# 10XGenomics/vartrix

Hardware: NVIDIA B200
Metric: reads_sw_scored_per_sec (higher is better)
Workload: dtype int16x2

## Files before the change

vartrix_b200/csrc/vtx_api.cu:

```cuda
#include "../../include/vartrix_b200.h"
#include "vtx_pipeline.cuh"
#include "vtx_sw.cuh"
#include "vtx_sw_band.cuh"
#include "vtx_inflate.cuh"
#include "vtx_stage.cuh"

#include <nvtx3/nvToolsExt.h>

#include <algorithm>
#include <cstdarg>
#include <cstdio>
#include <cstring>
#include <string>
#include <thread>
#include <vector>

using namespace vtx;

namespace {

thread_local std::string g_create_error;

struct Nvtx {
    explicit Nvtx(const char* name) { nvtxRangePushA(name); }
// ... 71 lines not shown
    void* h_res[7] = { nullptr, nullptr, nullptr, nullptr, nullptr, nullptr, nullptr };
    size_t h_res_cap = 0;
    void* h_scalars = nullptr;
    uint64_t last_n = 0;
    vtx_metrics last_metrics{};

    cudaStream_t fetch_stream = nullptr;
    unsigned long long* h_cum = nullptr;
    unsigned long long* d_cum = nullptr;
    std::vector<TimeRec> trecs;
    size_t trec_used = 0;
    bool timing_valid = false;
    uint32_t last_tiles_nl = 0;
    bool last_tiles_valid = false;
    uint64_t t_pairs = 0;

    void* comm = nullptr;
    int rank = 0, n_ranks = 1;
    void* g_host[7] = { nullptr, nullptr, nullptr, nullptr, nullptr, nullptr, nullptr };
    size_t g_host_cap = 0;
    DBuf g_dev[7];
    DBuf g_counts;
    cudaStream_t comm_stream = nullptr;
    cudaEvent_t ev_counts = nullptr, ev_gather = nullptr, ev_results = nullptr;
    uint64_t* h_counts = nullptr;
    bool gather_pending = false;
    bool gather_guard = false;
    vtx_result g_out{};
};

namespace {

int set_err(vtx_ctx* c, int code, const char* fmt, ...)
{
    char buf[512];
    va_list ap; va_start(ap, fmt); vsnprintf(buf, sizeof(buf), fmt, ap); va_end(ap);
    if (c) c->err = buf; else g_create_error = buf;
    return code;
}

#define CK(call)                                                                                     \
    do {                                                                                             \
        cudaError_t e_ = (call);                                                                     \
        if (e_ != cudaSuccess)                                                                       \
            return set_err(ctx, VTX_E_CUDA, "%s failed: %s (%s:%d)", #call, cudaGetErrorString(e_), __FILE__, __LINE__); \
    } while (0)

int ensure(vtx_ctx* ctx, DBuf& b, size_t bytes)
{
    if (bytes <= b.cap) return VTX_OK;
    if (b.p) {
        CK(cudaStreamSynchronize(ctx->stream));
        if (ctx->copy_stream) CK(cudaStreamSynchronize(ctx->copy_stream));
        CK(cudaFree(b.p)); b.p = nullptr; b.cap = 0;
    }
    size_t want = bytes + bytes / 8 + 256;
    cudaError_t e = cudaMalloc(&b.p, want);
    if (e != cudaSuccess) { b.p = nullptr; return set_err(ctx, VTX_E_NOMEM, "cudaMalloc(%zu) failed: %s", want, cudaGetErrorString(e)); }
    b.cap = want;
    return VTX_OK;
}

#define ENS(buf, bytes) do { int rc_ = ensure(ctx, buf, (bytes)); if (rc_) return rc_; } while (0)

template <typename T> T* P(DBuf& b) { return static_cast<T*>(b.p); }

TimeRec* new_trec(vtx_ctx* ctx)
{
    if (ctx->finished) ctx->trec_used = 0;
    if (ctx->trec_used == ctx->trecs.size()) {
        TimeRec r;
        for (auto& e : r.ev) if (cudaEventCreate(&e) != cudaSuccess) return nullptr;
        ctx->trecs.push_back(r);
    }
    TimeRec* r = &ctx->trecs[ctx->trec_used++];
    r->had_h2d = false; r->sw_launches = 0; r->launches = 0;
    return r;
}

inline unsigned blocks_for(uint64_t n, unsigned threads) { return unsigned((n + threads - 1) / threads); }

int scan_u32(vtx_ctx* ctx, const uint32_t* in, uint64_t n, uint32_t* out, uint64_t* launches)
{
    const unsigned nb = std::max(1u, blocks_for(n, kScanTile));
    ENS(ctx->scan_sums, size_t(nb) * 4);
    vtx_k_scan_tiles<<<nb, kScanThreads, 0, ctx->stream>>>(in, n, out, P<uint32_t>(ctx->scan_sums));
    vtx_k_scan_sums<<<1, kScanThreads, 0, ctx->stream>>>(P<uint32_t>(ctx->scan_sums), nb, out + n);
    vtx_k_scan_add<<<nb, kScanThreads, 0, ctx->stream>>>(out, n, P<uint32_t>(ctx->scan_sums));
    if (launches) *launches += 3;
    CK(cudaGetLastError());
    return VTX_OK;
}

struct DevBatch {
    uint32_t n_loci = 0; uint32_t n_reads = 0; uint64_t n_cand = 0;
    const uint32_t* locus_row; const uint8_t* hap; const uint32_t *ref_off, *ref_len, *alt_off, *alt_len;
    const uint64_t* cand_start; const uint8_t* read_nib; const uint64_t* read_off; const uint32_t* read_len;
    const uint8_t* cb_bytes; const uint32_t* read_cb_off; const uint16_t* read_cb_len; const uint64_t* read_umi;
    const uint32_t* cand_read;
    const uint64_t* read_cb_key = nullptr; const uint32_t* cb_off_ex = nullptr;
    uint32_t class_mask = ~0u;
    uint32_t max_read_len = 0, max_hap_len = 0;
    uint64_t max_depth = ~0ull;
};

struct SwAllow { bool split, multi, fold; };
SwAllow sw_allow(const vtx_ctx* ctx, uint32_t max_read, uint32_t max_hap)
{
    SwAllow a;
    a.split = max_read <= uint32_t(kSplitMaxRead) && !(ctx->cfg.flags & VTX_F_NO_SPLIT);
    a.multi = max_read <= uint32_t(kMultiMaxRead) && max_hap > uint32_t(class_max_n(kNumFastClasses - 1));
    a.fold = !(ctx->cfg.flags & (VTX_F_NO_SPLIT | VTX_F_NO_FOLD));
    return a;
}
template <int CLS>
int launch_sw_class(vtx_ctx* ctx, SwArgs a, uint64_t* launches)
{
    using TC = TileClass<CLS>;
    constexpr int PPW = 32 / TC::LPP, RS = TC::LPP * TC::CS;
    const size_t codes_bytes = (size_t(PPW) * (a.mcap + 2 * TC::LPP) * 2 + 7) & ~size_t(7);
    const size_t bnd_bytes = (CLS == kMultiClass && a.multi) ? size_t(PPW) * (a.mcap + 8) * 8 : 0;
    const size_t warp_bytes = (size_t(5 * RS) * 4 + codes_bytes + bnd_bytes + 15) & ~size_t(15);
    constexpr int kSwThreads = TC::THREADS;
    const size_t smem = warp_bytes * (kSwThreads / 32);
    auto kern = vtx_k_sw_pairs<CLS>;
    CK(cudaFuncSetAttribute(kern, cudaFuncAttributeMaxDynamicSharedMemorySize, int(smem)));
    int per_sm = 0;
    CK(cudaOccupancyMaxActiveBlocksPerMultiprocessor(&per_sm, kern, kSwThreads, smem));
    if (per_sm < 1) return set_err(ctx, VTX_E_CUDA, "SW kernel class %d does not fit on an SM (smem %zu)", CLS, smem);
    kern<<<ctx->n_sm * per_sm, kSwThreads, smem, ctx->stream>>>(a);
    CK(cudaGetLastError());
    ++*launches;
    return VTX_OK;
}

template <int SCLS>
int launch_sw_split(vtx_ctx* ctx, SwArgs a, uint64_t* launches)
{
    using SC = SplitClass<SCLS>;
    const size_t smem = split_warp_bytes<SCLS>(a.mcap) * (SC::THREADS / 32);
    auto kern = vtx_k_sw_split<SCLS>;
    CK(cudaFuncSetAttribute(kern, cudaFuncAttributeMaxDynamicSharedMemorySize, int(smem)));
    int per_sm = 0;
    CK(cudaOccupancyMaxActiveBlocksPerMultiprocessor(&per_sm, kern, SC::THREADS, smem));
    if (per_sm < 1) return set_err(ctx, VTX_E_CUDA, "split SW kernel %d does not fit on an SM (smem %zu)", SCLS, smem);
    kern<<<ctx->n_sm * per_sm, SC::THREADS, smem, ctx->stream>>>(a);
    CK(cudaGetLastError());
    ++*launches;
    return VTX_OK;
}

int launch_sw_fold(vtx_ctx* ctx, SwArgs a, uint64_t* launches)
{
    const size_t smem = fold_warp_bytes() * (kFoldThreads / 32);
    auto kern = vtx_k_sw_fold;
    CK(cudaFuncSetAttribute(kern, cudaFuncAttributeMaxDynamicSharedMemorySize, int(smem)));
    int per_sm = 0;
    CK(cudaOccupancyMaxActiveBlocksPerMultiprocessor(&per_sm, kern, kFoldThreads, smem));
    if (per_sm < 1) return set_err(ctx, VTX_E_CUDA, "folded SW kernel does not fit on an SM (smem %zu)", smem);
    kern<<<ctx->n_sm * per_sm, kFoldThreads, smem, ctx->stream>>>(a);
    CK(cudaGetLastError());
    ++*launches;
    return VTX_OK;
}

int run_sw(vtx_ctx* ctx, const DevBatch& b, uint32_t n_pairs_ub, const uint32_t* pair_slot, uint32_t* counters,
           uint32_t* pair_scores, uint64_t* launches, uint64_t* sw_launches, TimeRec* tr)
{
    const uint32_t nl = b.n_loci;
    ENS(ctx->tcount, size_t(kNumClasses) * (nl + 1) * 4);
    ENS(ctx->tstart, size_t(kNumClasses) * (nl + 1) * 4);
    ENS(ctx->tile_counters, 64);
    const int force_slow = 0;
    const SwAllow allow = sw_allow(ctx, b.max_read_len, b.max_hap_len);
    const int allow_split = allow.split, allow_multi = allow.multi, allow_fold = allow.fold;
    vtx_k_locus_prep<<<blocks_for(uint64_t(nl) * 32, 256), 256, 0, ctx->stream>>>(
        nl, b.hap, b.ref_off, b.ref_len, b.alt_off, b.alt_len, P<uint32_t>(ctx->pair_start), P<uint32_t>(ctx->pair_read), b.read_len,
        force_slow, allow_split, allow_multi, allow_fold, b.max_read_len, b.max_hap_len, P<unsigned long long>(ctx->d_metrics) + 4,
        P<uint32_t>(ctx->tcount));
    ++*launches;
    vtx_k_scan_rows<<<kNumClasses, kScanThreads, 0, ctx->stream>>>(P<uint32_t>(ctx->tcount), P<uint32_t>(ctx->tstart), nl, nl + 1);
    ++*launches;
    CK(cudaGetLastError());
    CK(cudaMemsetAsync(ctx->tile_counters.p, 0, 64, ctx->stream));
    ctx->last_tiles_nl = nl;
    ctx->last_tiles_valid = true;
    if (tr) CK(cudaEventRecord(tr->ev[EV_PREP], ctx->stream));

    SwArgs a{};
    a.hap_bytes = b.hap; a.ref_off = b.ref_off; a.ref_len = b.ref_len; a.alt_off = b.alt_off; a.alt_len = b.alt_len;
    a.read_nib = b.read_nib; a.read_off = b.read_off; a.read_len = b.read_len;
    a.pair_read = P<uint32_t>(ctx->pair_read); a.pair_start = P<uint32_t>(ctx->pair_start);
    a.n_loci = nl; a.pair_slot = pair_slot; a.counters = counters; a.pair_scores = pair_scores;
    a.min_score = ctx->cfg.min_score;
    int mcap = int(std::min<uint32_t>(b.max_read_len, kFastMaxRead));
    mcap = std::max(2, (mcap + 1) & ~1);
    a.mcap = mcap;
    a.k64k = 65536u;
    a.one = 1u;
    a.multi = allow_multi;
    a.max_hap = b.max_hap_len;

    uint64_t before = *launches;
    if (ctx->cfg.band_mode == VTX_BAND_MODEL) {
        BandArgs ba{};
        ba.sw = a; ba.n_pairs_ub = n_pairs_ub; ba.k = ctx->cfg.band_k; ba.w = ctx->cfg.band_w;
        ba.max_read = std::max<uint32_t>(b.max_read_len, 8); ba.max_hap = std::max<uint32_t>(b.max_hap_len, 8);
        const uint64_t all_hits = uint64_t(ba.max_read) * ba.max_hap;
        ba.hit_cap = uint32_t(std::min<uint64_t>(all_hits, uint64_t(1) << 20));
        ba.hit_cap = std::min<uint32_t>(ba.hit_cap, 65535u * 16u);
        const size_t wb = band_warp_bytes(ba.max_read, ba.max_hap, ba.hit_cap);
        size_t warps = size_t(ctx->n_sm) * 16;
        const size_t budget = size_t(4) << 30;
        if (warps * wb > budget) warps = std::max<size_t>(size_t(ctx->n_sm), budget / wb);
        warps = std::max<size_t>(warps & ~size_t(3), 4);
        ENS(ctx->band_scratch, warps * wb);
        ba.scratch = P<uint8_t>(ctx->band_scratch);
        if (ba.max_hap >= 65536u || ba.max_read >= 65536u) return set_err(ctx, VTX_E_UNSUPPORTED, "band model: reads and windows must be shorter than 65536");
        ba.overflow = P<unsigned long long>(ctx->d_metrics) + 5;
        ba.bounds_violated = P<unsigned long long>(ctx->d_metrics) + 4;
        ba.cursor = P<uint32_t>(ctx->tile_counters);
        vtx_k_sw_band<<<unsigned(warps / (kBandThreads / 32)), kBandThreads, 0, ctx->stream>>>(ba);
        CK(cudaGetLastError());
        ++*launches;
        *sw_launches += *launches - before;
        return VTX_OK;
    }
    for (int c = 0; c < kNumFastClasses; ++c) {
        if (c > 0 && b.max_hap_len <= uint32_t(class_max_n(c - 1))) continue;
        if (!(b.class_mask >> c & 1u)) continue;
        a.tile_start = P<uint32_t>(ctx->tstart) + size_t(c) * (nl + 1);
        a.tile_counter = P<uint32_t>(ctx->tile_counters) + c;
        int rc = VTX_OK;
        switch (c) {
        case 0: rc = launch_sw_class<0>(ctx, a, launches); break;
        case 1: rc = launch_sw_class<1>(ctx, a, launches); break;
        case 2: rc = launch_sw_class<2>(ctx, a, launches); break;
        case 3: rc = launch_sw_class<3>(ctx, a, launches); break;
        }
        if (rc) return rc;
    }
    if (allow_split) {
        for (int c = 0; c < kNumSplitClasses; ++c) {
            if (c > 0 && b.max_hap_len <= uint32_t(split_max_n(c - 1))) continue;
            if (!(b.class_mask >> (kSplitClass0 + c) & 1u)) continue;
            a.tile_start = P<uint32_t>(ctx->tstart) + size_t(kSplitClass0 + c) * (nl + 1);
            a.tile_counter = P<uint32_t>(ctx->tile_counters) + kSplitClass0 + c;
            int rc = c == 0 ? launch_sw_split<0>(ctx, a, launches) : launch_sw_split<1>(ctx, a, launches);
            if (rc) return rc;
        }
    }
    if (allow_fold && (b.class_mask >> kFoldClass & 1u)) {
        a.tile_start = P<uint32_t>(ctx->tstart) + size_t(kFoldClass) * (nl + 1);
        a.tile_counter = P<uint32_t>(ctx->tile_counters) + kFoldClass;
        int rc = launch_sw_fold(ctx, a, launches);
        if (rc) return rc;
    }
    if (b.class_mask >> kSlowClass & 1u) {
        const unsigned blocks = unsigned(ctx->n_sm) * 4, threads = 128;
        const size_t warps = size_t(blocks) * threads / 32;
        ENS(ctx->scratch, warps * (size_t(b.max_hap_len) + 1) * 32 * 4);
        a.scratch = P<uint32_t>(ctx->scratch);
        a.tile_start = P<uint32_t>(ctx->tstart) + size_t(kSlowClass) * (nl + 1);
        a.tile_counter = P<uint32_t>(ctx->tile_counters) + kSlowClass;
        vtx_k_sw_generic<<<blocks, threads, 0, ctx->stream>>>(a);
        CK(cudaGetLastError());
        ++*launches;
    }
    *sw_launches += *launches - before;
    (void)n_pairs_ub;
    return VTX_OK;
}

int grow_results(vtx_ctx* ctx, size_t need)
{
    if (need <= ctx->res_cap) return VTX_OK;
    const size_t ncap = need + need / 4 + 1024;
    DBuf* bufs[7] = { &ctx->r_row, &ctx->r_col, &ctx->r_ref, &ctx->r_alt, &ctx->r_unk, &ctx->r_val, &ctx->r_val2 };
    const size_t esz[7] = { 4, 4, 4, 4, 4, 8, 8 };
    for (int i = 0; i < 7; ++i) {
        void* np = nullptr;
        cudaError_t e = cudaMalloc(&np, ncap * esz[i]);
        if (e != cudaSuccess) return set_err(ctx, VTX_E_NOMEM, "result cudaMalloc(%zu) failed: %s", ncap * esz[i], cudaGetErrorString(e));
        if (bufs[i]->p && ctx->res_ub && !ctx->finished)
            CK(cudaMemcpyAsync(np, bufs[i]->p, ctx->res_ub * esz[i], cudaMemcpyDeviceToDevice, ctx->stream));
        if (bufs[i]->p) {
            CK(cudaStreamSynchronize(ctx->stream));
            if (ctx->fetch_stream) CK(cudaStreamSynchronize(ctx->fetch_stream));
            if (ctx->comm_stream) CK(cudaStreamSynchronize(ctx->comm_stream));
            CK(cudaFree(bufs[i]->p));
        }
        bufs[i]->p = np; bufs[i]->cap = ncap * esz[i];
    }
    ctx->res_cap = ncap;
    return VTX_OK;
}

int process_batch(vtx_ctx* ctx, const DevBatch& b, TimeRec* tr)
{
    const uint64_t nc = b.n_cand;
    const uint32_t nl = b.n_loci, nr = b.n_reads;
    const int use_umi = ctx->cfg.use_umi ? 1 : 0;
    uint64_t launches = 0, sw_launches = 0;
    cudaStream_t st = ctx->stream;

    if (ctx->finished) {
        CK(cudaMemsetAsync(ctx->d_res_n.p, 0, 8, st));
        CK(cudaMemsetAsync(ctx->d_metrics.p, 0, 48, st));
        ctx->res_ub = 0;
        ctx->finished = false;
    }
    int rc = grow_results(ctx, ctx->res_ub + nc);
    if (rc) return rc;
// ... 1345 lines not shown
```

vartrix_b200/csrc/vtx_sw.cuh:

```cuda
#pragma once
#include <cstdint>
#include <cuda_runtime.h>

namespace vtx {

constexpr int kMatch = 1, kMismatch = -5, kGapOpen = -5, kGapExtend = -1;
constexpr int kGoe = kGapOpen + kGapExtend;

__host__ __device__ constexpr uint32_t pack2(int lo, int hi)
{
    return (uint32_t(uint16_t(int16_t(hi))) << 16) | uint32_t(uint16_t(int16_t(lo)));
}
constexpr int kBias = 16384;
constexpr uint32_t kGE2 = pack2(kGapExtend, kGapExtend);
constexpr uint32_t kBIAS2 = pack2(kBias, kBias);
constexpr uint32_t kGOE2 = pack2(kBias + kGoe, kBias + kGoe);
constexpr uint32_t kNEG2 = pack2(0, 0);
constexpr uint32_t kGoeAdd = (uint32_t(uint16_t(int16_t(kGoe - 1))) << 16) | uint32_t(uint16_t(int16_t(kGoe)));
#ifndef VTX_SW_FUSE
#define VTX_SW_FUSE 1
#endif
#ifndef VTX_SW_HADD
#define VTX_SW_HADD 0
#endif
__device__ __forceinline__ uint32_t padd(uint32_t x, uint32_t one, uint32_t c)
{
    (void)one;
    return x + c;
}
__device__ __forceinline__ uint32_t hadd(uint32_t h, uint32_t one, int col)
{
#if VTX_SW_HADD == 1
    (void)col;
    return h * one + kGoeAdd;
#elif VTX_SW_HADD == 2
    return (col & 1) ? h + kGoeAdd : h * one + kGoeAdd;
#else
    (void)one; (void)col;
    return h + kGoeAdd;
#endif
}
__device__ __forceinline__ uint32_t sw_h(uint32_t diag, uint32_t one, uint32_t s, uint32_t f, uint32_t e)
{
#if VTX_SW_FUSE
    (void)one;
    return __vimax3_s16x2(__viaddmax_s16x2(diag, s, f), e, kBIAS2);
#else
    return __vmaxs2(__vimax3_s16x2(padd(diag, one, s), f, kBIAS2), e);
#endif
}
constexpr int kProfMatch = kMatch - kGoe, kProfMis = kMismatch - kGoe;

constexpr int kFastMaxRead = 1024;
constexpr int kMaxRead = 16000;
constexpr int kNumFastClasses = 4;
constexpr int kSlowClass = kNumFastClasses;
constexpr int kNumSplitClasses = 2;
constexpr int kSplitClass0 = kSlowClass + 1;
constexpr int kFoldClass = kSplitClass0 + kNumSplitClasses;
constexpr int kNumClasses = kFoldClass + 1;
constexpr int kTileChunk = 8;

template <int CLS> struct TileClass;
template <> struct TileClass<0> { static constexpr int LPP = 8, C = 26, CS = 28, THREADS = 320, MINB = 2; };
template <> struct TileClass<1> { static constexpr int LPP = 8, C = 29, CS = 36, THREADS = 320, MINB = 2; };
template <> struct TileClass<2> { static constexpr int LPP = 8, C = 32, CS = 36, THREADS = 256, MINB = 2; };
template <> struct TileClass<3> { static constexpr int LPP = 8, C = 40, CS = 44, THREADS = 384, MINB = 1; };
constexpr int kMultiClass = 3;
constexpr int kMultiMaxRead = 256;
__host__ __device__ constexpr int class_max_n(int cls)
{
    return cls == 0 ? 208 : cls == 1 ? 232 : cls == 2 ? 256 : cls == 3 ? 320 : 0x7fffffff;
}
constexpr int kSlowPairsPerWarp = 16;

struct SwArgs {
    const uint8_t* hap_bytes;
    const uint32_t* ref_off; const uint32_t* ref_len; const uint32_t* alt_off; const uint32_t* alt_len;
    const uint8_t* read_nib; const uint64_t* read_off; const uint32_t* read_len;
    const uint32_t* pair_read;
    const uint32_t* pair_start;
    const uint32_t* tile_start;
    uint32_t n_loci;
    uint32_t* tile_counter;
    const uint32_t* pair_slot;
    uint32_t* counters;
    uint32_t* pair_scores;
    int32_t min_score;
    int32_t mcap;
    uint32_t k64k;
    uint32_t one;
    int32_t multi;
    uint32_t* scratch;
    uint32_t max_hap;
};

__device__ __forceinline__ uint32_t hap_code(uint8_t b)
{
    return b == 'A' ? 0u : b == 'C' ? 1u : b == 'G' ? 2u : b == 'T' ? 3u : 5u;
}
__device__ __forceinline__ uint32_t nib_code(uint32_t nib)
{
    return (0x4444444344424104ull >> (nib * 4)) & 0xF;
}

__device__ __forceinline__ uint32_t upper_locus(const uint32_t* __restrict__ a, uint32_t n, uint32_t v)
{
    uint32_t lo = 0, hi = n;
    while (hi - lo > 1) {
        uint32_t mid = (lo + hi) >> 1;
        if (__ldg(a + mid) <= v) lo = mid; else hi = mid;
    }
    return lo;
}

__device__ __forceinline__ void call_and_scatter(const SwArgs& a, uint32_t pair, uint32_t packed)
{
    const int ref_score = int(int16_t(packed & 0xFFFF)), alt_score = int(int16_t(packed >> 16));
    if (a.pair_scores) a.pair_scores[pair] = pack2(ref_score, alt_score);
    if (!a.pair_slot) return;
    if (ref_score < a.min_score && alt_score < a.min_score) return;
    const uint32_t k = ref_score > alt_score ? 0u : (alt_score > ref_score ? 1u : 2u);
    atomicAdd(a.counters + size_t(a.pair_slot[pair]) * 4 + k, 1u);
}

template <int CLS>
__global__ void __launch_bounds__(TileClass<CLS>::THREADS, TileClass<CLS>::MINB) vtx_k_sw_pairs(const SwArgs a)
{
    using TC = TileClass<CLS>;
    constexpr int LPP = TC::LPP, C = TC::C, CS = TC::CS;
    constexpr int PPW = 32 / LPP;
    constexpr int RS = LPP * CS;
    constexpr int M = LPP;
    static_assert(CS % 4 == 0 && ((CS / 4) & 1) == 1 && CS >= C, "bank-conflict-free stride");
    static_assert(RS % 32 == 0, "row stride keeps lanes on their banks");
    constexpr uint32_t kSentinel = 4u * RS * 4u;

    extern __shared__ __align__(16) uint8_t smem_raw[];
    const int lane = threadIdx.x & 31, warp = threadIdx.x >> 5;
    const int g = lane % LPP, grp = lane / LPP;
    constexpr bool MULTI = (CLS == kMultiClass);
    const int code_stride = a.mcap + 2 * M;
    const int bnd_stride = (MULTI && a.multi) ? a.mcap + 8 : 0;
    const size_t codes_bytes = (size_t(PPW) * code_stride * 2 + 7) & ~size_t(7);
    const size_t warp_bytes = size_t(5 * RS) * 4 + codes_bytes + size_t(PPW) * bnd_stride * 8;
    uint8_t* wbase = smem_raw + warp * ((warp_bytes + 15) & ~size_t(15));
    uint32_t* prof = reinterpret_cast<uint32_t*>(wbase);
    uint16_t* codes = reinterpret_cast<uint16_t*>(wbase + size_t(5 * RS) * 4) + grp * code_stride;
    uint2* bnd = reinterpret_cast<uint2*>(wbase + size_t(5 * RS) * 4 + codes_bytes) + grp * bnd_stride;

    const uint32_t n_tiles = __ldg(a.tile_start + a.n_loci);
    uint32_t cached_locus = 0xFFFFFFFFu;
    const uint32_t tile_chunk = max(1u, min(uint32_t(kTileChunk), n_tiles / (gridDim.x * (blockDim.x >> 5) * 16u)));

    for (;;) {
        uint32_t chunk = 0;
        if (lane == 0) chunk = atomicAdd(a.tile_counter, 1u);
        chunk = __shfl_sync(0xffffffffu, chunk, 0);
        const uint32_t t_begin = chunk * tile_chunk;
        if (t_begin >= n_tiles) break;
        const uint32_t t_end = min(t_begin + tile_chunk, n_tiles);

        uint32_t locus = upper_locus(a.tile_start, a.n_loci, t_begin);
        for (uint32_t tile = t_begin; tile < t_end; ++tile) {
            while (tile >= __ldg(a.tile_start + locus + 1)) ++locus;
            const uint32_t p0 = __ldg(a.pair_start + locus) + PPW * (tile - __ldg(a.tile_start + locus));
            const uint32_t p_end = __ldg(a.pair_start + locus + 1);

            __syncwarp();
            const uint8_t* rh = a.hap_bytes + __ldg(a.ref_off + locus);
            const uint8_t* ah = a.hap_bytes + __ldg(a.alt_off + locus);
            const int n_ref = int(__ldg(a.ref_len + locus)), n_alt = int(__ldg(a.alt_len + locus));
            const int n_pass = MULTI ? max(1, (max(n_ref, n_alt) + LPP * C - 1) / (LPP * C)) : 1;
            auto build_profile = [&](int col0) {
                for (int idx = lane; idx < RS; idx += 32) {
                    const int gg = idx / CS, k = idx - gg * CS;
                    const int j = col0 + gg * C + k;
                    uint32_t rb = 5, ab = 5;
                    if (k < C) {
                        if (j < n_ref) rb = hap_code(__ldg(rh + j));
                        if (j < n_alt) ab = hap_code(__ldg(ah + j));
                    }
#pragma unroll
                    for (uint32_t r = 0; r < 5; ++r)
                        prof[r * RS + idx] = pack2(r == rb ? kProfMatch : kProfMis, r == ab ? kProfMatch : kProfMis);
                }
            };
            if (n_pass == 1 && locus != cached_locus) { cached_locus = locus; build_profile(0); }
            if (n_pass > 1) cached_locus = 0xFFFFFFFFu;
            const uint32_t pair = p0 + grp;
            const bool active = pair < p_end;
            int m = 0;
            const uint8_t* nib = nullptr;
            if (active) {
                const uint32_t r = __ldg(a.pair_read + pair);
                m = int(__ldg(a.read_len + r));
                nib = a.read_nib + __ldg(a.read_off + r);
            }
            const int R = a.mcap;
            auto fill_codes = [&](int t0) {
                for (int e = g; e < code_stride; e += LPP) {
                    const int row = t0 - M + e;
                    uint32_t off = kSentinel;
                    if (row >= 0 && row < m) {
                        const uint32_t by = __ldg(nib + (row >> 1));
                        off = nib_code((row & 1) ? (by & 0xF) : (by >> 4)) * (RS * 4);
                    }
                    codes[e] = uint16_t(off);
                }
            };
            int mmax = m;
#pragma unroll
            for (int o = 16; o >= 1; o >>= 1) mmax = max(mmax, __shfl_xor_sync(0xffffffffu, mmax, o));

            uint32_t best = kBIAS2;
            const uint8_t* lane_prof = reinterpret_cast<const uint8_t*>(prof) + g * CS * 4;
            const uint16_t* my_codes = codes + M - g;
            const int steps = mmax + LPP - 1;
            const uint32_t one = a.one;
            for (int pass = 0; pass < n_pass; ++pass) {
                if (MULTI && n_pass > 1) { __syncwarp(); build_profile(pass * LPP * C); __syncwarp(); }
                uint32_t hg[C], f[C];
#pragma unroll
                for (int c = 0; c < C; ++c) { hg[c] = kGOE2; f[c] = kNEG2; }
                uint32_t hg_last = kGOE2, e_last = kNEG2, diag_save = kGOE2;
                for (int t0 = 0; t0 < steps; t0 += R) {
                __syncwarp();
                fill_codes(t0);
                __syncwarp();
                const int t_hi = min(steps, t0 + R);
                for (int t = t0; t < t_hi; ++t) {
                    uint32_t hl = __shfl_up_sync(0xffffffffu, hg_last, 1, LPP);
                    uint32_t el = __shfl_up_sync(0xffffffffu, e_last, 1, LPP);
                    if (g == 0) {
                        hl = kGOE2; el = kNEG2;
                        if (MULTI && pass > 0 && t < mmax) { const uint2 b = bnd[t]; hl = b.x; el = b.y; }
                    }
                    const uint4* prow = reinterpret_cast<const uint4*>(lane_prof + my_codes[t - t0]);
                    uint32_t diag = diag_save;
                    diag_save = hl;
                    uint32_t e = el, eg = hl, hleft = hl;
#pragma unroll
                    for (int q = 0; q < (C + 3) / 4; ++q) {
                        const uint4 s4 = prow[q];
                        const uint32_t sv[4] = { s4.x, s4.y, s4.z, s4.w };
// ... 84 lines not shown
```

vartrix_b200/csrc/vtx_sw_fold.cuh:

```cuda
#pragma once
#include "vtx_sw.cuh"

namespace vtx {

constexpr int kFoldP = 96;
constexpr int kFoldC1 = 12;
constexpr int kFoldPPW = 4;
constexpr int kFoldR = 19;
constexpr int kFoldMaxRead = 8 * kFoldR;
constexpr int kFoldMaxMid = 40;
constexpr int kFoldRows = kFoldMaxRead + 4;
constexpr int kFoldCodeStride = kFoldMaxRead + 16;
#ifndef VTX_FOLD_UNROLL
#define VTX_FOLD_UNROLL 2
#endif
#ifndef VTX_FOLD_PRESHIFT
#define VTX_FOLD_PRESHIFT 0
#endif
#ifndef VTX_FOLD_THREADS
#define VTX_FOLD_THREADS 288
#endif
constexpr int kFoldThreads = VTX_FOLD_THREADS;
constexpr int kFoldUnroll = VTX_FOLD_UNROLL;
#ifndef VTX_FOLD_MID_UNROLL
#define VTX_FOLD_MID_UNROLL 1
#endif
constexpr int kFoldMidUnroll = VTX_FOLD_MID_UNROLL;

__host__ __device__ constexpr size_t fold_warp_bytes()
{
    size_t b = size_t(2 * 5 * kFoldP) * 4;
    b += size_t(kFoldMaxMid) * 8 * 4;
    b += size_t(kFoldPPW) * kFoldRows * 8 + 32;
    b += size_t(2 * kFoldPPW) * kFoldCodeStride;
    return (b + 15) & ~size_t(15);
}

constexpr int kJuncH = -2 * kGoe - kBias, kJuncE = -kGapOpen - kBias;
constexpr uint32_t kJuncH2 = (uint32_t(uint16_t(int16_t(kJuncH - 1))) << 16) | uint32_t(uint16_t(int16_t(kJuncH)));
constexpr uint32_t kJuncE2 = (uint32_t(uint16_t(int16_t(kJuncE - 1))) << 16) | uint32_t(uint16_t(int16_t(kJuncE)));

__global__ void __launch_bounds__(kFoldThreads, 2) vtx_k_sw_fold(const SwArgs a)
{
    constexpr int C1 = kFoldC1, P = kFoldP, R = kFoldR, M = 8;
    constexpr int RS1 = P;

    extern __shared__ __align__(16) uint8_t smem_raw[];
    const int lane = threadIdx.x & 31, warp = threadIdx.x >> 5;
    const int u = lane >> 3, g = lane & 7;
    uint8_t* wbase = smem_raw + warp * fold_warp_bytes();
    uint32_t* profF = reinterpret_cast<uint32_t*>(wbase);
    uint32_t* profR = profF + 5 * RS1;
    uint32_t* midtab = profR + 5 * RS1;
    uint2* bnd = reinterpret_cast<uint2*>(midtab + kFoldMaxMid * 8);
    uint8_t* codes = reinterpret_cast<uint8_t*>(bnd + kFoldPPW * kFoldRows + 4);

    const uint32_t n_tiles = __ldg(a.tile_start + a.n_loci);
    uint32_t cached_locus = 0xFFFFFFFFu;
    const uint32_t tile_chunk = max(1u, min(uint32_t(kTileChunk), n_tiles / (gridDim.x * (blockDim.x >> 5) * 16u)));
    const uint32_t k64k = a.k64k;
    const uint32_t one = a.one;
    int mid_ref = 0, mid_alt = 0;

    for (;;) {
        uint32_t chunk = 0;
        if (lane == 0) chunk = atomicAdd(a.tile_counter, 1u);
        chunk = __shfl_sync(0xffffffffu, chunk, 0);
        const uint32_t t_begin = chunk * tile_chunk;
        if (t_begin >= n_tiles) break;
        const uint32_t t_end = min(t_begin + tile_chunk, n_tiles);
        uint32_t locus = upper_locus(a.tile_start, a.n_loci, t_begin);
        for (uint32_t tile = t_begin; tile < t_end; ++tile) {
            while (tile >= __ldg(a.tile_start + locus + 1)) ++locus;
            const uint32_t p0 = __ldg(a.pair_start + locus) + kFoldPPW * (tile - __ldg(a.tile_start + locus));
            const uint32_t p_end = __ldg(a.pair_start + locus + 1);
            __syncwarp();
            if (locus != cached_locus) {
                cached_locus = locus;
                const uint8_t* rh = a.hap_bytes + __ldg(a.ref_off + locus);
                const uint8_t* ah = a.hap_bytes + __ldg(a.alt_off + locus);
                const int n_ref = int(__ldg(a.ref_len + locus)), n_alt = int(__ldg(a.alt_len + locus));
                mid_ref = n_ref - 2 * P;
                mid_alt = n_alt - 2 * P;
                for (int j = lane; j < P; j += 32) {
                    const uint32_t fb = hap_code(__ldg(rh + j));
                    const uint32_t sb = hap_code(__ldg(rh + (n_ref - 1 - j)));
#pragma unroll
                    for (uint32_t r = 0; r < 5; ++r) {
                        profF[r * RS1 + j] = uint32_t(r == fb ? kProfMatch : kProfMis);
                        profR[r * RS1 + j] = uint32_t(r == sb ? kProfMatch : kProfMis) << (VTX_FOLD_PRESHIFT ? 16 : 0);
                    }
                }
                const int lmax = max(mid_ref, mid_alt);
                for (int idx = lane; idx < lmax * 8; idx += 32) {
                    const int k = idx >> 3;
                    const uint32_t r = uint32_t(idx & 7);
                    const uint32_t rb = k < mid_ref ? hap_code(__ldg(rh + P + k)) : 5u;
                    const uint32_t ab = k < mid_alt ? hap_code(__ldg(ah + P + k)) : 5u;
                    midtab[idx] = pack2(r == rb ? kProfMatch : kProfMis, r == ab ? kProfMatch : kProfMis);
                }
            }
            const uint32_t pair = p0 + u;
            const bool active = pair < p_end;
            int m = 0;
            {
                const uint8_t* nib = nullptr;
                if (active) {
                    const uint32_t rd = __ldg(a.pair_read + pair);
                    m = int(__ldg(a.read_len + rd));
                    nib = a.read_nib + __ldg(a.read_off + rd);
                }
                uint8_t* cf = codes + (2 * u) * kFoldCodeStride;
                uint8_t* cr = cf + kFoldCodeStride;
                for (int e = g; e < kFoldCodeStride; e += 8)
                    if (e < M || e >= M + m) { cf[e] = 4; cr[e] = 4; }
                for (int b = g; 2 * b < m; b += 8) {
                    const uint32_t by = __ldg(nib + b);
                    const uint8_t c0 = uint8_t(nib_code(by >> 4)), c1 = uint8_t(nib_code(by & 0xF));
                    cf[M + 2 * b] = c0;
                    cr[M + m - 1 - 2 * b] = c0;
                    if (2 * b + 1 < m) { cf[M + 2 * b + 1] = c1; cr[M + m - 2 - 2 * b] = c1; }
                }
            }
            int mmax = m;
#pragma unroll
            for (int o = 16; o >= 1; o >>= 1) mmax = max(mmax, __shfl_xor_sync(0xffffffffu, mmax, o));
            __syncwarp();

            uint2* my_bnd = bnd + u * kFoldRows;
            const uint2* row_bnd = my_bnd + 7;
            uint32_t best;
            {
                uint32_t hg[C1], f[C1];
#pragma unroll
                for (int c = 0; c < C1; ++c) { hg[c] = kGOE2; f[c] = kNEG2; }
                uint32_t hg_last = kGOE2, e_last = kNEG2, diag_save = kGOE2;
                best = kBIAS2;
                const uint8_t* cA = codes + (2 * u) * kFoldCodeStride + M - g;
                const uint8_t* cB = cA + kFoldCodeStride;
                const uint32_t* lane_f = profF + g * C1;
                const uint32_t* lane_r = profR + g * C1;
                const int steps = mmax + 7;
#pragma unroll kFoldUnroll
                for (int t = 0; t < steps; ++t) {
                    uint32_t hl = __shfl_up_sync(0xffffffffu, hg_last, 1, 8);
                    uint32_t el = __shfl_up_sync(0xffffffffu, e_last, 1, 8);
                    if (g == 0) { hl = kGOE2; el = kNEG2; }
                    const uint4* pa = reinterpret_cast<const uint4*>(lane_f + uint32_t(cA[t]) * RS1);
                    const uint4* pb = reinterpret_cast<const uint4*>(lane_r + uint32_t(cB[t]) * RS1);
                    uint32_t diag = diag_save;
                    diag_save = hl;
                    uint32_t e = el, eg = hl, hleft = hl;
#pragma unroll
                    for (int q = 0; q < C1 / 4; ++q) {
                        const uint4 a4 = pa[q], b4 = pb[q];
#if VTX_FOLD_PRESHIFT
                        const uint32_t sv[4] = { b4.x + a4.x, b4.y + a4.y, b4.z + a4.z, b4.w + a4.w };
#else
                        const uint32_t sv[4] = { b4.x * k64k + a4.x, b4.y * k64k + a4.y, b4.z * k64k + a4.z, b4.w * k64k + a4.w };
#endif
                        uint32_t hh[4];
#pragma unroll
                        for (int k = 0; k < 4; ++k) {
                            const int c = 4 * q + k;
                            const uint32_t fc = __viaddmax_s16x2(f[c], kGE2, hg[c]);
                            e = __viaddmax_s16x2(e, kGE2, eg);
                            const uint32_t h = sw_h(diag, one, sv[k], fc, e);
                            hh[k] = h;
                            diag = hg[c];
                            hleft = hadd(h, one, c);
                            eg = hleft;
                            hg[c] = hleft;
                            f[c] = fc;
                        }
                        best = __vimax3_s16x2(best, hh[0], hh[1]);
                        best = __vimax3_s16x2(best, hh[2], hh[3]);
                    }
                    hg_last = hleft;
                    e_last = e;
                    if (g == 7) my_bnd[t] = make_uint2(hleft, e);
                }
#pragma unroll
                for (int o = 4; o >= 1; o >>= 1) best = __vmaxs2(best, __shfl_xor_sync(0xffffffffu, best, o));
                best = __vmaxs2(best, __byte_perm(best, 0, 0x1032));
            }
            __syncwarp();

            {
                const int lmax = max(mid_ref, mid_alt), lmin = min(mid_ref, mid_alt);
                const uint32_t short_mask = mid_ref < mid_alt ? 0x0000FFFFu : 0xFFFF0000u;
                uint32_t hg[R], e[R], rc[R];
                const uint8_t* cf = codes + (2 * u) * kFoldCodeStride + M + R * g;
#pragma unroll
                for (int c = 0; c < R; ++c) {
                    const int row = R * g + c;
                    uint2 b = make_uint2(kGOE2, kNEG2);
                    if (row < mmax) b = row_bnd[row];
                    hg[c] = __byte_perm(b.x, 0, 0x1010);
                    e[c] = __byte_perm(b.y, 0, 0x1010);
                    rc[c] = uint32_t(cf[c]) * 4u;
                }
                auto junction = [&](uint32_t mask) {
                    uint32_t cross = kBIAS2;
#pragma unroll
                    for (int c = 0; c < R; ++c) {
                        const int rr = m - 2 - (R * g + c);
                        uint2 b = make_uint2(kGOE2, kGOE2);
                        if (rr >= 0) b = row_bnd[rr];
                        const uint32_t ph = __byte_perm(b.x, 0, 0x3232), pe = __byte_perm(b.y, 0, 0x3232);
                        const uint32_t x1 = hg[c] + ph + kJuncH2;
                        const uint32_t x2 = e[c] + pe + kJuncE2;
                        cross = __vimax3_s16x2(cross, x1, x2);
                    }
                    best = __vmaxs2(best, (cross & mask) | (kBIAS2 & ~mask));
                };
                uint32_t diag_save = kGOE2;
                if (g > 0 && R * g - 1 < mmax) diag_save = __byte_perm(row_bnd[R * g - 1].x, 0, 0x1010);
                uint32_t hup_last = kGOE2, f_last = kNEG2;
                const uint8_t* tab = reinterpret_cast<const uint8_t*>(midtab) - 32 * g;
                const int steps = lmax + 7;
#pragma unroll kFoldMidUnroll
                for (int s = 0; s < steps; ++s) {
                    uint32_t hup = __shfl_up_sync(0xffffffffu, hup_last, 1, 8);
                    uint32_t fup = __shfl_up_sync(0xffffffffu, f_last, 1, 8);
                    if (g == 0) { hup = kGOE2; fup = kNEG2; }
                    const int k = s - g;
                    if (k >= 0 && k < lmax) {
                        const uint8_t* trow = tab + 32 * s;
                        uint32_t diag = diag_save;
                        diag_save = hup;
                        uint32_t f = fup, fg = hup, hdown = hup;
                        uint32_t hh[2];
#pragma unroll
                        for (int c = 0; c < R; ++c) {
                            const uint32_t sv = *reinterpret_cast<const uint32_t*>(trow + rc[c]);
                            const uint32_t ec = __viaddmax_s16x2(e[c], kGE2, hg[c]);
                            f = __viaddmax_s16x2(f, kGE2, fg);
                            const uint32_t h = sw_h(diag, one, sv, ec, f);
                            hh[c & 1] = h;
                            diag = hg[c];
                            hdown = hadd(h, one, c);
                            fg = hdown;
                            hg[c] = hdown;
                            e[c] = ec;
                            if (c & 1) best = __vimax3_s16x2(best, hh[0], hh[1]);
                        }
                        if (R & 1) best = __vmaxs2(best, hh[0]);
                        hup_last = hdown;
                        f_last = f;
                        if (k == lmin - 1 && lmin != lmax) junction(short_mask);
                    }
                }
                junction(lmin != lmax ? ~short_mask : 0xFFFFFFFFu);
#pragma unroll
                for (int o = 4; o >= 1; o >>= 1) best = __vmaxs2(best, __shfl_xor_sync(0xffffffffu, best, o));
                if (active && g == 0) call_and_scatter(a, pair, best - kBIAS2);
            }
        }
    }
}

}
```

Measured before the change: 157.1 million.

## Fuse forward/reverse profiles into paired 16-row table and pack code pairs

```diff
diff --git a/vartrix_b200/csrc/vtx_api.cu b/vartrix_b200/csrc/vtx_api.cu
--- a/vartrix_b200/csrc/vtx_api.cu
+++ b/vartrix_b200/csrc/vtx_api.cu
@@ -247,13 +247,19 @@
 
 int launch_sw_fold(vtx_ctx* ctx, SwArgs a, uint64_t* launches)
 {
-    const size_t smem = fold_warp_bytes() * (kFoldThreads / 32);
+    a.fold_mid_cap = std::min(std::max(int(a.max_hap) - 2 * kFoldP, 1), kFoldMaxMid);
+    const size_t wb = fold_warp_bytes(a.fold_mid_cap);
     auto kern = vtx_k_sw_fold;
-    CK(cudaFuncSetAttribute(kern, cudaFuncAttributeMaxDynamicSharedMemorySize, int(smem)));
-    int per_sm = 0;
-    CK(cudaOccupancyMaxActiveBlocksPerMultiprocessor(&per_sm, kern, kFoldThreads, smem));
+    CK(cudaFuncSetAttribute(kern, cudaFuncAttributeMaxDynamicSharedMemorySize, int(wb * (kFoldThreads / 32))));
+    int threads = kFoldThreads, per_sm = 0;
+    CK(cudaOccupancyMaxActiveBlocksPerMultiprocessor(&per_sm, kern, threads, wb * (threads / 32)));
+    if (per_sm < 2) {
+        threads = kFoldThreadsNarrow;
+        CK(cudaOccupancyMaxActiveBlocksPerMultiprocessor(&per_sm, kern, threads, wb * (threads / 32)));
+    }
+    const size_t smem = wb * (threads / 32);
     if (per_sm < 1) return set_err(ctx, VTX_E_CUDA, "folded SW kernel does not fit on an SM (smem %zu)", smem);
-    kern<<<ctx->n_sm * per_sm, kFoldThreads, smem, ctx->stream>>>(a);
+    kern<<<ctx->n_sm * per_sm, threads, smem, ctx->stream>>>(a);
     CK(cudaGetLastError());
     ++*launches;
     return VTX_OK;
diff --git a/vartrix_b200/csrc/vtx_sw.cuh b/vartrix_b200/csrc/vtx_sw.cuh
--- a/vartrix_b200/csrc/vtx_sw.cuh
+++ b/vartrix_b200/csrc/vtx_sw.cuh
@@ -91,6 +91,7 @@
     uint32_t k64k;
     uint32_t one;
     int32_t multi;
+    int32_t fold_mid_cap;
     uint32_t* scratch;
     uint32_t max_hap;
 };
diff --git a/vartrix_b200/csrc/vtx_sw_fold.cuh b/vartrix_b200/csrc/vtx_sw_fold.cuh
--- a/vartrix_b200/csrc/vtx_sw_fold.cuh
+++ b/vartrix_b200/csrc/vtx_sw_fold.cuh
@@ -9,30 +9,28 @@
 constexpr int kFoldR = 19;
 constexpr int kFoldMaxRead = 8 * kFoldR;
 constexpr int kFoldMaxMid = 40;
+constexpr int kFoldProfRows = 17;
+constexpr uint8_t kFoldSentinel = 16;
+constexpr uint8_t kFoldSentinelMixed = 4 << 3 | 4;
 constexpr int kFoldRows = kFoldMaxRead + 4;
 constexpr int kFoldCodeStride = kFoldMaxRead + 16;
 #ifndef VTX_FOLD_UNROLL
 #define VTX_FOLD_UNROLL 2
 #endif
-#ifndef VTX_FOLD_PRESHIFT
-#define VTX_FOLD_PRESHIFT 0
-#endif
-#ifndef VTX_FOLD_THREADS
-#define VTX_FOLD_THREADS 288
-#endif
-constexpr int kFoldThreads = VTX_FOLD_THREADS;
+constexpr int kFoldThreads = 288;
+constexpr int kFoldThreadsNarrow = 256;
 constexpr int kFoldUnroll = VTX_FOLD_UNROLL;
 #ifndef VTX_FOLD_MID_UNROLL
 #define VTX_FOLD_MID_UNROLL 1
 #endif
 constexpr int kFoldMidUnroll = VTX_FOLD_MID_UNROLL;
 
-__host__ __device__ constexpr size_t fold_warp_bytes()
-{
-    size_t b = size_t(2 * 5 * kFoldP) * 4;
-    b += size_t(kFoldMaxMid) * 8 * 4;
+__host__ __device__ inline size_t fold_warp_bytes(int mid_cap)
+{
+    size_t b = size_t(kFoldProfRows * kFoldP) * 4;
+    b += size_t(mid_cap) * 8 * 4;
     b += size_t(kFoldPPW) * kFoldRows * 8 + 32;
-    b += size_t(2 * kFoldPPW) * kFoldCodeStride;
+    b += size_t(kFoldPPW) * kFoldCodeStride;
     return (b + 15) & ~size_t(15);
 }
 
@@ -40,25 +38,88 @@
 constexpr uint32_t kJuncH2 = (uint32_t(uint16_t(int16_t(kJuncH - 1))) << 16) | uint32_t(uint16_t(int16_t(kJuncH)));
 constexpr uint32_t kJuncE2 = (uint32_t(uint16_t(int16_t(kJuncE - 1))) << 16) | uint32_t(uint16_t(int16_t(kJuncE)));
 
+__device__ __forceinline__ uint32_t lop_lo_hi(uint32_t a, uint32_t b)
+{
+    uint32_t d;
+    asm("lop3.b32 %0, %1, %2, %3, 0xE2;" : "=r"(d) : "r"(a), "r"(0x0000FFFFu), "r"(b));
+    return d;
+}
+
+template <bool MIXED>
+__device__ __forceinline__ uint32_t fold_main_pass(const uint32_t* __restrict__ prof, const uint8_t* __restrict__ cA, int steps,
+                                                   int g, uint32_t one, uint2* __restrict__ my_bnd)
+{
+    constexpr int C1 = kFoldC1, RS1 = kFoldP;
+    uint32_t hg[C1], f[C1];
+#pragma unroll
+    for (int c = 0; c < C1; ++c) { hg[c] = kGOE2; f[c] = kNEG2; }
+    uint32_t hg_last = kGOE2, e_last = kNEG2, diag_save = kGOE2;
+    uint32_t best = kBIAS2;
+    const uint32_t* lane_p = prof + g * C1;
+#pragma unroll kFoldUnroll
+    for (int t = 0; t < steps; ++t) {
+        uint32_t hl = __shfl_up_sync(0xffffffffu, hg_last, 1, 8);
+        uint32_t el = __shfl_up_sync(0xffffffffu, e_last, 1, 8);
+        if (g == 0) { hl = kGOE2; el = kNEG2; }
+        const uint32_t code = cA[t];
+        const uint4* pa = reinterpret_cast<const uint4*>(lane_p + (MIXED ? (code >> 3) * 4 : code) * RS1);
+        const uint4* pb = reinterpret_cast<const uint4*>(lane_p + ((code & 7) + 3 * (code & 4)) * RS1);
+        uint32_t diag = diag_save;
+        diag_save = hl;
+        uint32_t e = el, eg = hl, hleft = hl;
+#pragma unroll
+        for (int q = 0; q < C1 / 4; ++q) {
+            uint32_t sv[4];
+            const uint4 a4 = pa[q];
+            if (MIXED) {
+                const uint4 b4 = pb[q];
+                sv[0] = lop_lo_hi(a4.x, b4.x); sv[1] = lop_lo_hi(a4.y, b4.y);
+                sv[2] = lop_lo_hi(a4.z, b4.z); sv[3] = lop_lo_hi(a4.w, b4.w);
+            } else {
+                sv[0] = a4.x; sv[1] = a4.y; sv[2] = a4.z; sv[3] = a4.w;
+            }
+            uint32_t hh[4];
+#pragma unroll
+            for (int k = 0; k < 4; ++k) {
+                const int c = 4 * q + k;
+                const uint32_t fc = __viaddmax_s16x2(f[c], kGE2, hg[c]);
+                e = __viaddmax_s16x2(e, kGE2, eg);
+                const uint32_t h = sw_h(diag, one, sv[k], fc, e);
+                hh[k] = h;
+                diag = hg[c];
+                hleft = hadd(h, one, c);
+                eg = hleft;
+                hg[c] = hleft;
+                f[c] = fc;
+            }
+            best = __vimax3_s16x2(best, hh[0], hh[1]);
+            best = __vimax3_s16x2(best, hh[2], hh[3]);
+        }
+        hg_last = hleft;
+        e_last = e;
+        if (g == 7) my_bnd[t] = make_uint2(hleft, e);
+    }
+    return best;
+}
+
 __global__ void __launch_bounds__(kFoldThreads, 2) vtx_k_sw_fold(const SwArgs a)
 {
-    constexpr int C1 = kFoldC1, P = kFoldP, R = kFoldR, M = 8;
+    constexpr int P = kFoldP, R = kFoldR, M = 8;
     constexpr int RS1 = P;
 
     extern __shared__ __align__(16) uint8_t smem_raw[];
     const int lane = threadIdx.x & 31, warp = threadIdx.x >> 5;
     const int u = lane >> 3, g = lane & 7;
-    uint8_t* wbase = smem_raw + warp * fold_warp_bytes();
-    uint32_t* profF = reinterpret_cast<uint32_t*>(wbase);
-    uint32_t* profR = profF + 5 * RS1;
-    uint32_t* midtab = profR + 5 * RS1;
-    uint2* bnd = reinterpret_cast<uint2*>(midtab + kFoldMaxMid * 8);
+    const int mid_cap = a.fold_mid_cap;
+    uint8_t* wbase = smem_raw + warp * fold_warp_bytes(mid_cap);
+    uint32_t* prof = reinterpret_cast<uint32_t*>(wbase);
+    uint32_t* midtab = prof + kFoldProfRows * RS1;
+    uint2* bnd = reinterpret_cast<uint2*>(midtab + mid_cap * 8);
     uint8_t* codes = reinterpret_cast<uint8_t*>(bnd + kFoldPPW * kFoldRows + 4);
 
     const uint32_t n_tiles = __ldg(a.tile_start + a.n_loci);
     uint32_t cached_locus = 0xFFFFFFFFu;
     const uint32_t tile_chunk = max(1u, min(uint32_t(kTileChunk), n_tiles / (gridDim.x * (blockDim.x >> 5) * 16u)));
-    const uint32_t k64k = a.k64k;
     const uint32_t one = a.one;
     int mid_ref = 0, mid_alt = 0;
 
@@ -86,10 +147,9 @@
                     const uint32_t fb = hap_code(__ldg(rh + j));
                     const uint32_t sb = hap_code(__ldg(rh + (n_ref - 1 - j)));
 #pragma unroll
-                    for (uint32_t r = 0; r < 5; ++r) {
-                        profF[r * RS1 + j] = uint32_t(r == fb ? kProfMatch : kProfMis);
-                        profR[r * RS1 + j] = uint32_t(r == sb ? kProfMatch : kProfMis) << (VTX_FOLD_PRESHIFT ? 16 : 0);
-                    }
+                    for (uint32_t p = 0; p < 16; ++p)
+                        prof[p * RS1 + j] = pack2((p >> 2) == fb ? kProfMatch : kProfMis, (p & 3) == sb ? kProfMatch : kProfMis);
+                    prof[16 * RS1 + j] = pack2(kProfMis, kProfMis);
                 }
                 const int lmax = max(mid_ref, mid_alt);
                 for (int idx = lane; idx < lmax * 8; idx += 32) {
@@ -103,6 +163,8 @@
             const uint32_t pair = p0 + u;
             const bool active = pair < p_end;
             int m = 0;
+            uint8_t* cw = codes + u * kFoldCodeStride;
+            bool mixed;
             {
                 const uint8_t* nib = nullptr;
                 if (active) {
@@ -110,17 +172,23 @@
                     m = int(__ldg(a.read_len + rd));
                     nib = a.read_nib + __ldg(a.read_off + rd);
                 }
-                uint8_t* cf = codes + (2 * u) * kFoldCodeStride;
-                uint8_t* cr = cf + kFoldCodeStride;
-                for (int e = g; e < kFoldCodeStride; e += 8)
-                    if (e < M || e >= M + m) { cf[e] = 4; cr[e] = 4; }
+                bool other = false;
                 for (int b = g; 2 * b < m; b += 8) {
                     const uint32_t by = __ldg(nib + b);
-                    const uint8_t c0 = uint8_t(nib_code(by >> 4)), c1 = uint8_t(nib_code(by & 0xF));
-                    cf[M + 2 * b] = c0;
-                    cr[M + m - 1 - 2 * b] = c0;
-                    if (2 * b + 1 < m) { cf[M + 2 * b + 1] = c1; cr[M + m - 2 - 2 * b] = c1; }
-                }
+                    const uint32_t c0 = nib_code(by >> 4), c1 = nib_code(by & 0xF);
+                    cw[M + 2 * b] = uint8_t(c0);
+                    other |= c0 == 4;
+                    if (2 * b + 1 < m) { cw[M + 2 * b + 1] = uint8_t(c1); other |= c1 == 4; }
+                }
+                mixed = __any_sync(0xffffffffu, other);
+                __syncwarp();
+                for (int i = g; 2 * i < m; i += 8) {
+                    const uint32_t x = cw[M + i], y = cw[M + m - 1 - i];
+                    cw[M + i] = uint8_t(mixed ? x << 3 | y : 4 * x + y);
+                    cw[M + m - 1 - i] = uint8_t(mixed ? y << 3 | x : 4 * y + x);
+                }
+                for (int e = g; e < kFoldCodeStride; e += 8)
+                    if (e < M || e >= M + m) cw[e] = mixed ? kFoldSentinelMixed : kFoldSentinel;
             }
             int mmax = m;
 #pragma unroll
@@ -129,68 +197,19 @@
 
             uint2* my_bnd = bnd + u * kFoldRows;
             const uint2* row_bnd = my_bnd + 7;
-            uint32_t best;
-            {
-                uint32_t hg[C1], f[C1];
-#pragma unroll
-                for (int c = 0; c < C1; ++c) { hg[c] = kGOE2; f[c] = kNEG2; }
-                uint32_t hg_last = kGOE2, e_last = kNEG2, diag_save = kGOE2;
-                best = kBIAS2;
-                const uint8_t* cA = codes + (2 * u) * kFoldCodeStride + M - g;
-                const uint8_t* cB = cA + kFoldCodeStride;
-                const uint32_t* lane_f = profF + g * C1;
-                const uint32_t* lane_r = profR + g * C1;
-                const int steps = mmax + 7;
-#pragma unroll kFoldUnroll
-                for (int t = 0; t < steps; ++t) {
-                    uint32_t hl = __shfl_up_sync(0xffffffffu, hg_last, 1, 8);
-                    uint32_t el = __shfl_up_sync(0xffffffffu, e_last, 1, 8);
-                    if (g == 0) { hl = kGOE2; el = kNEG2; }
-                    const uint4* pa = reinterpret_cast<const uint4*>(lane_f + uint32_t(cA[t]) * RS1);
-                    const uint4* pb = reinterpret_cast<const uint4*>(lane_r + uint32_t(cB[t]) * RS1);
-                    uint32_t diag = diag_save;
-                    diag_save = hl;
-                    uint32_t e = el, eg = hl, hleft = hl;
-#pragma unroll
-                    for (int q = 0; q < C1 / 4; ++q) {
-                        const uint4 a4 = pa[q], b4 = pb[q];
-#if VTX_FOLD_PRESHIFT
-                        const uint32_t sv[4] = { b4.x + a4.x, b4.y + a4.y, b4.z + a4.z, b4.w + a4.w };
-#else
-                        const uint32_t sv[4] = { b4.x * k64k + a4.x, b4.y * k64k + a4.y, b4.z * k64k + a4.z, b4.w * k64k + a4.w };
-#endif
-                        uint32_t hh[4];
-#pragma unroll
-                        for (int k = 0; k < 4; ++k) {
-                            const int c = 4 * q + k;
-                            const uint32_t fc = __viaddmax_s16x2(f[c], kGE2, hg[c]);
-                            e = __viaddmax_s16x2(e, kGE2, eg);
-                            const uint32_t h = sw_h(diag, one, sv[k], fc, e);
-                            hh[k] = h;
-                            diag = hg[c];
-                            hleft = hadd(h, one, c);
-                            eg = hleft;
-                            hg[c] = hleft;
-                            f[c] = fc;
-                        }
-                        best = __vimax3_s16x2(best, hh[0], hh[1]);
-                        best = __vimax3_s16x2(best, hh[2], hh[3]);
-                    }
-                    hg_last = hleft;
-                    e_last = e;
-                    if (g == 7) my_bnd[t] = make_uint2(hleft, e);
-                }
-#pragma unroll
-                for (int o = 4; o >= 1; o >>= 1) best = __vmaxs2(best, __shfl_xor_sync(0xffffffffu, best, o));
-                best = __vmaxs2(best, __byte_perm(best, 0, 0x1032));
-            }
+            uint32_t best = mixed ? fold_main_pass<true>(prof, cw + M - g, mmax + 7, g, one, my_bnd)
+                                  : fold_main_pass<false>(prof, cw + M - g, mmax + 7, g, one, my_bnd);
+#pragma unroll
+            for (int o = 4; o >= 1; o >>= 1) best = __vmaxs2(best, __shfl_xor_sync(0xffffffffu, best, o));
+            best = __vmaxs2(best, __byte_perm(best, 0, 0x1032));
             __syncwarp();
 
             {
                 const int lmax = max(mid_ref, mid_alt), lmin = min(mid_ref, mid_alt);
                 const uint32_t short_mask = mid_ref < mid_alt ? 0x0000FFFFu : 0xFFFF0000u;
                 uint32_t hg[R], e[R], rc[R];
-                const uint8_t* cf = codes + (2 * u) * kFoldCodeStride + M + R * g;
+                const uint8_t* cf = cw + M + R * g;
+                const uint32_t fwd_shift = mixed ? 3 : 2;
 #pragma unroll
                 for (int c = 0; c < R; ++c) {
                     const int row = R * g + c;
@@ -198,7 +217,7 @@
                     if (row < mmax) b = row_bnd[row];
                     hg[c] = __byte_perm(b.x, 0, 0x1010);
                     e[c] = __byte_perm(b.y, 0, 0x1010);
-                    rc[c] = uint32_t(cf[c]) * 4u;
+                    rc[c] = (uint32_t(cf[c]) >> fwd_shift) * 4u;
                 }
                 auto junction = [&](uint32_t mask) {
                     uint32_t cross = kBIAS2;
```

Measured after the change: 173.1 million (median of 6 runs). 1.1x the previous value.
